# uc-vision/taichi_gaussian_rasterizer

Measured on AMD Instinct MI355X. Metric: Mpixels/s fwd+bwd @ 2048x2048, 1M Gaussians, higher is better.
Workload: dtype f32

## Files before the change

taichi_gaussian_rasterizer_amd/csrc/frame.cpp:

```cpp

#include <string.h>

#include "gs_common.h"

namespace {

int64_t a256(int64_t bytes) { return gs_align_up(bytes > 0 ? bytes : 1, 256); }

struct Dims {
  int64_t n, P, T;
  int C, F, col0, RS, tiles_x, tiles_y, local_h, D;
  bool want_vis;
};

int frame_dims(const GsFrame* f, Dims* d) {
  GS_REQUIRE(f != nullptr, GS_ERR_INVALID_ARGUMENT, "frame: descriptor is NULL");
  if (int rc = gs_check_cfg(&f->cfg)) return rc;
  GS_REQUIRE(f->n >= 0 && f->n < (int64_t(1) << 31), GS_ERR_INVALID_ARGUMENT, "frame: %lld gaussians", (long long)f->n);
  GS_REQUIRE(f->width > 0 && f->height > 0, GS_ERR_INVALID_ARGUMENT, "frame: image size %dx%d", f->width, f->height);
  GS_REQUIRE(f->sh_degree >= -1 && f->sh_degree <= 3, GS_ERR_UNSUPPORTED, "frame: SH degree %d", f->sh_degree);
  GS_REQUIRE(f->channels >= 1 && f->channels <= (f->sh_degree >= 0 ? GS_MAX_SH_CHANNELS : GS_MAX_FEATURES - 2),
             GS_ERR_UNSUPPORTED, "frame: %d feature channels", f->channels);
  const int ts = f->cfg.tile_size;
  GsShard sh;
// ... 130 lines not shown
  int32_t* tile_order = at<int32_t>(workspace, L.tile_order);
  int32_t* o2p = at<int32_t>(workspace, L.overlap_to_point);
  float* image = at<float>(workspace, L.image);
  float* alpha = at<float>(workspace, L.alpha);
  float* vis = L.visibility >= 0 ? at<float>(workspace, L.visibility) : nullptr;
  float* ndc = at<float>(scratch, L.s_ndc_depth);
  void* stage = at<char>(scratch, L.s_stage);
  const int64_t map_bytes = gs_map_scratch_bytes(d.n, d.T > 0 ? d.T : 1);
  void* proj_stage = at<char>(stage, a256(map_bytes));
  const int64_t proj_bytes = L.stage_bytes - a256(map_bytes);

  const bool lists = shard && f->exchange_world > 0 && d.T > 0;
  GS_REQUIRE(f->exchange_world <= 64 && (f->exchange_world == 0 || (f->exchange_rank >= 0 && f->exchange_rank < f->exchange_world)),
             GS_ERR_INVALID_ARGUMENT, "gs_frame_fwd: exchange rank %d of %d", f->exchange_rank, f->exchange_world);
  if (lists && f->sh_degree >= 0 &&
      hipMemsetD32Async(reinterpret_cast<hipDeviceptr_t>(feats), 0x3F000000, size_t(d.n) * d.F, s) != hipSuccess) {
    gs_set_error("gs_frame_fwd: hipMemsetD32Async failed");
    return GS_ERR_LAUNCH;
  }
  GsMapBinPlan bin;
  bin.width = f->width; bin.height = f->height; bin.cfg = cfg; bin.shard = shard; bin.scratch = stage;
  bin.scratch_bytes = map_bytes;
  tm.mark(GS_FWD_PROJECT, 0, stream);
  if (int rc = gs_project_fwd_ex(d.n, position, log_scaling, rotation, alpha_logit, T_camera_world, projection,
                                 f->width, f->height, f->near_plane, f->far_plane, cfg, points, depth, ndc, indexes,
                                 slot_of, counts, f->render_depth ? feats : nullptr, d.F, cam_pos, proj_stage,
                                 proj_bytes, L.grad_rows >= 0 ? at<float>(workspace, L.grad_rows) : nullptr, d.RS,
                                 d.T > 0 ? &bin : nullptr, stream))
    return rc;
  tm.mark(GS_FWD_PROJECT, 1, stream);
  const int32_t* v_dev = counts;
  float* colours = feats + d.col0;
  int rc;
  tm.mark(GS_FWD_COLOURS, 0, stream);
  if (f->sh_degree >= 0 && lists)
    rc = GS_OK;
  else if (f->sh_degree >= 0 && shard)
    rc = gs_sh_fwd_shard(d.n, v_dev, d.C, f->sh_degree, feature, position, indexes, cam_pos, points, f->height, cfg,
                         shard, colours, d.F, stream);
  else if (f->sh_degree >= 0)
    rc = gs_sh_fwd(d.n, v_dev, d.C, f->sh_degree, feature, position, indexes, cam_pos, colours, d.F, stream);
  else
    rc = gs_feature_gather_fwd(d.n, v_dev, d.C, feature, indexes, colours, d.F, stream);
  tm.mark(GS_FWD_COLOURS, 1, stream);
  if (rc) return rc;
  if (vis && hipMemsetAsync(vis, 0, size_t(d.n) * 4, s) != hipSuccess) {
    gs_set_error("gs_frame_fwd: hipMemsetAsync failed");
    return GS_ERR_LAUNCH;
  }
  if (d.T == 0) {
    if (hipMemsetAsync(counts + 1, 0, 28, s) != hipSuccess) { gs_set_error("gs_frame_fwd: memset failed"); return GS_ERR_LAUNCH; }
    if (L.owner_counts >= 0 && hipMemsetAsync(at<char>(workspace, L.owner_counts), 0, 64 * 8, s) != hipSuccess) {
      gs_set_error("gs_frame_fwd: memset failed");
      return GS_ERR_LAUNCH;
    }
    if (counts_host) {
      if (hipMemcpyAsync(counts_host, counts + 4, 16, hipMemcpyDeviceToHost, s) != hipSuccess ||
          hipMemcpyAsync(counts_host + 4, counts, 4, hipMemcpyDeviceToHost, s) != hipSuccess ||
          hipMemcpyAsync(counts_host + 5, counts + 5, 4, hipMemcpyDeviceToHost, s) != hipSuccess) {
        gs_set_error("gs_frame_fwd: count read-back failed");
        return GS_ERR_LAUNCH;
      }
    }
    if (counts_event && hipEventRecord(static_cast<hipEvent_t>(counts_event), s) != hipSuccess) {
      gs_set_error("gs_frame_fwd: hipEventRecord failed");
      return GS_ERR_LAUNCH;
    }
    return tm.rc;
  }
  tm.mark(GS_FWD_MAP_PREPARE, 0, stream);
  if ((rc = gs_map_prepare_ex(d.n, v_dev, points, f->width, f->height, cfg, f->k_capacity, tile_ranges, counts + 4,
                              counts_host, tile_order, shard, stage, map_bytes, 1, stream)))
    return rc;
  tm.mark(GS_FWD_MAP_PREPARE, 1, stream);
  if (counts_event && hipEventRecord(static_cast<hipEvent_t>(counts_event), s) != hipSuccess) {
    gs_set_error("gs_frame_fwd: hipEventRecord failed");
    return GS_ERR_LAUNCH;
  }
  if (lists) {
    int32_t* touched = at<int32_t>(workspace, L.touched);
    if ((rc = gs_map_touched_list(d.n, v_dev, d.T, stage, map_bytes, touched, counts + 1, indexes, d.n,
                                  f->exchange_world, at<int64_t>(workspace, L.owner_counts), f->exchange_rank,
                                  counts + 2, stream)))
      return rc;
    if (f->sh_degree >= 0) {
      tm.mark(GS_FWD_COLOURS, 0, stream);
      if ((rc = gs_sh_fwd_rows(d.n, touched, counts + 1, d.C, f->sh_degree, feature, position, indexes, cam_pos, colours,
                               d.F, stream)))
        return rc;
      tm.mark(GS_FWD_COLOURS, 1, stream);
    }
  }
  const int32_t tile_hint = f->max_tile_hint > 0 ? -f->max_tile_hint : 0;
  tm.mark(GS_FWD_MAP_FINISH, 0, stream);
  if ((rc = gs_map_finish(d.n, v_dev, f->k_capacity, tile_hint, points, ndc, f->width, f->height, cfg, f->use_depth16,
                          tile_ranges, o2p, nullptr, at<char>(scratch, L.s_pairs), shard, stage, map_bytes,
                          stream)))
    return rc;
  tm.mark(GS_FWD_MAP_FINISH, 1, stream);
  tm.mark(GS_FWD_RASTER, 0, stream);
  if ((rc = gs_raster_fwd(d.n, d.F, points, feats, tile_ranges, o2p, f->k_capacity, f->width, f->height, &rcfg,
                          tile_order, counts + 7, image, alpha, vis, shard, stream)))
    return rc;
  tm.mark(GS_FWD_RASTER, 1, stream);
  if (f->render_depth &&
// ... 101 lines not shown
```

taichi_gaussian_rasterizer_amd/csrc/gs_common.h:

```cpp
#pragma once

#include <hip/hip_runtime.h>
#include <stdint.h>
#include <stdio.h>

#include "../../include/gsplat_hip.h"

#define GS_WAVE 64

void gs_set_error(const char* fmt, ...);

#define GS_REQUIRE(cond, status, ...)  \
  do {                                 \
    if (!(cond)) {                     \
      gs_set_error(__VA_ARGS__);       \
      return (status);                 \
    }                                  \
  } while (0)

#define GS_CHECK_LAUNCH(name)                                                   \
  do {                                                                          \
    hipError_t e_ = hipGetLastError();                                          \
    if (e_ != hipSuccess) {                                                     \
      gs_set_error("%s: launch failed: %s", name, hipGetErrorString(e_));       \
// ... 73 lines not shown

int gs_raster_sub_blocks(const GsRasterConfig* cfg, int64_t num_tiles, int backward);

int gs_project_fwd_ex(int64_t n, const float* position, const float* log_scaling, const float* rotation,
                      const float* alpha_logit, const float* T_camera_world, const float* projection, int32_t width,
                      int32_t height, double near_plane, double far_plane, const GsRasterConfig* cfg, float* points,
                      float* depth, float* ndc_depth, int64_t* indexes, int32_t* slot_of, int32_t* num_visible,
                      float* depth_features, int32_t depth_features_stride, float* camera_pos, void* scratch,
                      int64_t scratch_bytes, float* zero_rows, int32_t zero_row_floats, const struct GsMapBinPlan* bin,
                      void* stream);
struct GsMapBinPlan {
  int32_t width, height;
  const GsRasterConfig* cfg;
  const GsRowShard* shard;
  void* scratch;
  int64_t scratch_bytes;
};
struct GsCompactArgs {
  int64_t n;
  const void* st_rows;
  const int* block_offsets;
  const int* block_counts;
  int num_blocks;
  float inv_far, ndc_denom;
  float* points; float* depth; float* ndc; int64_t* indexes; int* slot_of; int* num_visible;
  float* depth_feat; int depth_feat_stride;
  void* zero_rows; int zero_row_v4;
};
int gs_map_compact_bin(const GsMapBinPlan* plan, const GsCompactArgs* c, void* stream);
int gs_map_bin_counters(const GsMapBinPlan* plan, int64_t n, int32_t** words, int32_t* count);
int64_t gs_map_one_pass_scratch_bytes(int64_t n);
int gs_map_project_compact_bin(const GsMapBinPlan* plan, const void* pa, const GsCompactArgs* c, float* camera_pos,
                               void* lookback, void* stream);
int gs_map_prepare_ex(int64_t v, const int32_t* v_dev, const float* points, int32_t width, int32_t height,
                      const GsRasterConfig* cfg, int64_t k_capacity, int32_t* tile_ranges, int32_t* counts_out,
                      int32_t* counts_host, int32_t* tile_order, const GsRowShard* shard, void* scratch,
                      int64_t scratch_bytes, int binned, void* stream);
int gs_rows_add(int64_t v, int32_t row_floats, float* rows, const float* add_points, const float* add_depth,
                int32_t depth_col, void* stream);

#ifdef __HIPCC__

__device__ __forceinline__ int gs_xcd_remap(int block, int n) {
  const int chunk = (n + 7) >> 3;
  const int item = (block & 7) * chunk + (block >> 3);
  return ((block >> 3) < chunk && item < n) ? item : -1;
}

template <int CTRL, int ROW_MASK = 0xf, int BANK_MASK = 0xf>
__device__ __forceinline__ float gs_dpp_add(float x) {
  const int moved = __builtin_amdgcn_update_dpp(0, __float_as_int(x), CTRL, ROW_MASK, BANK_MASK, false);
  return x + __int_as_float(moved);
}

__device__ __forceinline__ float gs_wave_sum_to_lane63(float x) {
  x = gs_dpp_add<0x128>(x);
  x = gs_dpp_add<0x124>(x);
  x = gs_dpp_add<0x122>(x);
  x = gs_dpp_add<0x121>(x);
  x = gs_dpp_add<0x142, 0xa>(x);
  x = gs_dpp_add<0x143, 0xc>(x);
  return x;
}

template <int CTRL>
__device__ __forceinline__ float gs_dpp_add_full(float x) {
  return x + __int_as_float(__builtin_amdgcn_mov_dpp(__float_as_int(x), CTRL, 0xf, 0xf, true));
}

__device__ __forceinline__ float gs_wave_reduce16_transposed(float (&v)[16], int lane) {
// ... 176 lines not shown
```

taichi_gaussian_rasterizer_amd/csrc/mapper.hip:

```cpp

#include "gs_common.h"
#include "../../include/gs_detmath.h"
#include "project_math.h"

namespace {

struct GridQuery {
  float ib00, ib01, ib10, ib11;
  float rel_min_x, rel_min_y;
  int min_tx, min_ty, span_x, span_y;
};

__device__ __forceinline__ GridQuery grid_query(const float* g, int Wp, int Hp, int tile_size, float alpha_thr) {
  GridQuery q;
  const float mx = g[0], my = g[1], ax = g[2], ay = g[3], sgx = g[4], sgy = g[5], alpha = g[6];
  if (!(alpha > alpha_thr)) {
    q.ib00 = q.ib01 = q.ib10 = q.ib11 = q.rel_min_x = q.rel_min_y = 0.f;
    q.min_tx = q.min_ty = q.span_x = q.span_y = 0;
    return q;
  }
  const float gscale = gs_det_sqrtf(2.0f * gs_det_logf(__fdiv_rn(alpha, alpha_thr)));
  const float sx = sgx * gscale, sy = sgy * gscale;
  const float a2x = -ay, a2y = ax;
  const float v1x = ax * sx, v1y = ay * sx, v2x = a2x * sy, v2y = a2y * sy;
  const float ex = gs_det_sqrtf(v1x * v1x + v2x * v2x), ey = gs_det_sqrtf(v1y * v1y + v2y * v2y);
  const float lox = mx - ex, loy = my - ey, hix = mx + ex, hiy = my + ey;
  q.ib00 = __fdiv_rn(ax, sx); q.ib01 = __fdiv_rn(ay, sx); q.ib10 = __fdiv_rn(a2x, sy); q.ib11 = __fdiv_rn(a2y, sy);
  const float ts = float(tile_size);
  const int max_tx = (Wp - 1) / tile_size, max_ty = (Hp - 1) / tile_size;
  int min_tx = int(floorf(__fdiv_rn(lox, ts))), min_ty = int(floorf(__fdiv_rn(loy, ts)));
  min_tx = max(min_tx, 0); min_ty = max(min_ty, 0);
  int hi_tx = int(ceilf(__fdiv_rn(hix, ts))), hi_ty = int(ceilf(__fdiv_rn(hiy, ts)));
  hi_tx = min(max(hi_tx, min_tx + 1), max_tx + 1);
  hi_ty = min(max(hi_ty, min_ty + 1), max_ty + 1);
  q.min_tx = min_tx; q.min_ty = min_ty;
  q.span_x = max(hi_tx - min_tx, 0); q.span_y = max(hi_ty - min_ty, 0);
// ... 45 lines not shown
__device__ __forceinline__ int64_t live_count(const MapArgs& a) {
  if (a.v_dev == nullptr) return a.v;
  const int64_t d = *a.v_dev;
  return d < a.v ? d : a.v;
}

__device__ __forceinline__ int wave_inclusive_scan(int x) {
  x += __builtin_amdgcn_update_dpp(0, x, 0x111, 0xf, 0xf, true);
  x += __builtin_amdgcn_update_dpp(0, x, 0x112, 0xf, 0xf, true);
  x += __builtin_amdgcn_update_dpp(0, x, 0x114, 0xf, 0xf, true);
  x += __builtin_amdgcn_update_dpp(0, x, 0x118, 0xf, 0xf, true);
  x += __builtin_amdgcn_update_dpp(0, x, 0x142, 0xa, 0xf, false);
  x += __builtin_amdgcn_update_dpp(0, x, 0x143, 0xc, 0xf, false);
  return x;
}

__device__ __forceinline__ int block_exclusive_scan(int x, int* s_wave, int& sum) {
  const int lane = threadIdx.x & 63, wv = threadIdx.x >> 6;
  const int inc = wave_inclusive_scan(x);
  if (lane == 63) s_wave[wv] = inc;
  __syncthreads();
  int before = 0;
  sum = 0;
#pragma unroll
  for (int w = 0; w < 16; ++w) {
    const int tot = s_wave[w];
    sum += tot;
    before += w < wv ? tot : 0;
  }
  __syncthreads();
  return before + inc - x;
}

__global__ __launch_bounds__(1024) void map_scan_kernel(int num_tiles, const int* tile_hist, int2* tile_ranges,
                                                        int* cursors, int* counts_out, int64_t k_capacity,
                                                        int* tile_order, const int* v_dev, int* counts_host,
                                                        const int* touched_dev) {
  __shared__ int s_wave[16];
  __shared__ int s_bin[1024];
  const int t = threadIdx.x;
  if (blockIdx.x == 0) {
    constexpr int PER = 16;
    int carry = 0, mx = 0;
    for (int base0 = 0; base0 < num_tiles; base0 += 1024 * PER) {
      const int i0 = base0 + t * PER;
      int c[PER];
      const bool whole = i0 + PER <= num_tiles;
      if (whole) {
        const int4* src = reinterpret_cast<const int4*>(tile_hist + i0);
#pragma unroll
        for (int q = 0; q < PER / 4; ++q) {
          const int4 v4 = src[q];
          c[4 * q] = v4.x; c[4 * q + 1] = v4.y; c[4 * q + 2] = v4.z; c[4 * q + 3] = v4.w;
        }
      } else {
#pragma unroll
        for (int j = 0; j < PER; ++j) c[j] = i0 + j < num_tiles ? tile_hist[i0 + j] : 0;
      }
      int sum = 0;
#pragma unroll
      for (int j = 0; j < PER; ++j) { sum += c[j]; mx = max(mx, c[j]); }
      int total;
      int run = carry + block_exclusive_scan(sum, s_wave, total);
      carry += total;
      int2 rg[PER];
      int cur[PER];
#pragma unroll
      for (int j = 0; j < PER; ++j) {
        const bool fits = k_capacity <= 0 || int64_t(run) + c[j] <= k_capacity;
        rg[j] = (c[j] > 0 && fits) ? make_int2(run, run + c[j]) : make_int2(0, 0);
// ... 130 lines not shown
__device__ __forceinline__ void publish_region_hist(const int* s_hist, const RegionGrid& rg, int num_wg, int blk,
                                                    int* part, int* region_count) {
  for (int r = threadIdx.x; r < rg.num_regions; r += BIN) {
    const int h = s_hist[r];
    if (region_count == nullptr) part[int64_t(r) * num_wg + blk] = h;
    else if (h > 0) part[int64_t(r) * num_wg + blk] = atomicAdd(region_count + r, h);
  }
}
__global__ __launch_bounds__(BIN) void region_count_kernel(MapArgs a, RegionGrid rg, int num_wg, int* region_of,
                                                           int* part, int* touched_blocks, int* block_start,
                                                           int* region_count) {
  __shared__ int s_hist[MAX_REGIONS];
  for (int r = threadIdx.x; r < rg.num_regions; r += BIN) s_hist[r] = 0;
  __syncthreads();
  const int64_t i = int64_t(blockIdx.x) * BIN + threadIdx.x;
  bool mine = false;
  const int64_t live = live_count(a);
  if (threadIdx.x == 0) {
    block_start[blockIdx.x] = int(min(int64_t(blockIdx.x) * BIN, live));
    if (int(blockIdx.x) == num_wg - 1) block_start[num_wg] = int(live);
  }
  if (i < live) {
    const bool any = enters_order(a.points + 7 * i, a);
    const int r = any ? region_of_gaussian(a.points + 7 * i, a, rg) : -1;
    region_of[i] = r;
    if (r >= 0) atomicAdd(&s_hist[r], 1);
    mine = r >= 0;
  }
  const int touched = __syncthreads_count(mine);
  if (threadIdx.x == 0) touched_blocks[blockIdx.x] = touched;
  publish_region_hist(s_hist, rg, num_wg, blockIdx.x, part, region_count);
}

__global__ __launch_bounds__(1024) void region_part_scan_kernel(int num_wg, int* part, int* region_count,
                                                                int) {
  __shared__ int s_wave[16];
  int* row = part + int64_t(blockIdx.x) * num_wg;
  int carry = 0;
  for (int base = 0; base < num_wg; base += 1024) {
    const int i = base + threadIdx.x;
    const int v = i < num_wg ? row[i] : 0;
    int total;
    const int before = block_exclusive_scan(v, s_wave, total);
    if (i < num_wg) row[i] = carry + before;
    carry += total;
  }
  if (threadIdx.x == 0) region_count[blockIdx.x] = carry;
}

__global__ __launch_bounds__(1024) void region_scan_kernel(int num_regions, const int* region_count, int* region_start,
                                                           int* chunk_start) {
  __shared__ int s_wave[16];
  const int r = threadIdx.x;
  const int c = r < num_regions ? region_count[r] : 0;
  const int ch = (c + CHUNK - 1) / CHUNK;
  int total_c, total_ch;
  const int start = block_exclusive_scan(c, s_wave, total_c);
  const int chunk = block_exclusive_scan(ch, s_wave, total_ch);
  if (r < num_regions) {
    region_start[r] = start;
    chunk_start[r] = chunk;
  }
  if (r == 0) {
    region_start[num_regions] = total_c;
    chunk_start[num_regions] = total_ch;
  }
}

__global__ __launch_bounds__(BIN) void region_scatter_kernel(RegionGrid rg, int num_wg, const int* region_of,
                                                             const int* part, const int* region_count,
                                                             int* region_start, int* chunk_start,
                                                             const int* block_start, int* order, int* tile_hist,
                                                             int num_tiles, int scanned) {
  __shared__ int s_cnt[MAX_REGIONS];
  __shared__ int s_start[MAX_REGIONS];
  __shared__ int s_wave[16];
  for (int i = blockIdx.x * BIN + threadIdx.x; i < num_tiles; i += gridDim.x * BIN) tile_hist[i] = 0;
  const int t = threadIdx.x;
  s_cnt[t] = 0;
  if (scanned) {
    s_start[t] = t < rg.num_regions ? region_start[t] : 0;
  } else {
    const int c = t < rg.num_regions ? region_count[t] : 0;
    int total_c;
// ... 1075 lines not shown
  const MapScratch m = carve(plan->scratch, c->n, num_tiles);
  const unsigned vb = unsigned(gs_div_up(c->n, BIN));
  hipStream_t s = static_cast<hipStream_t>(stream);
  int* counters = bin_with_atomics(vb, rg) ? m.region_count : nullptr;
  if (counters && hipMemsetAsync(counters, 0, size_t(MAX_REGIONS + 1) * 4, s) != hipSuccess) {
    gs_set_error("gs_map_project_compact_bin: hipMemsetAsync failed");
    return GS_ERR_LAUNCH;
  }
  if (c->block_offsets == reinterpret_cast<const int*>(1)) {
    GsCompactArgs c2 = *c;
    c2.block_offsets = nullptr;
    c2.block_counts = static_cast<int*>(lookback);
    hipLaunchKernelGGL(project_count_kernel, dim3(vb), dim3(BIN), 0, s, *static_cast<const gs_proj::ProjArgs*>(pa),
                       static_cast<int*>(lookback));
    hipLaunchKernelGGL(project_compact_bin_kernel<false>, dim3(vb), dim3(BIN), 0, s,
                       *static_cast<const gs_proj::ProjArgs*>(pa), c2, a, rg, int(vb), m.region_of, m.part,
                       m.touched_blocks, m.block_start, counters, nullptr, nullptr, nullptr, camera_pos);
    GS_CHECK_LAUNCH("gs_map_project_compact_bin");
    return GS_OK;
  }
  if (hipMemsetAsync(lookback, 0, size_t(gs_map_one_pass_scratch_bytes(c->n)), s) != hipSuccess) {
    gs_set_error("gs_map_project_compact_bin: hipMemsetAsync failed");
    return GS_ERR_LAUNCH;
  }
  unsigned long long* desc = static_cast<unsigned long long*>(lookback);
  int* ticket = reinterpret_cast<int*>(desc + vb);
  hipLaunchKernelGGL(project_compact_bin_kernel<true>, dim3(vb), dim3(BIN), 0, s,
                     *static_cast<const gs_proj::ProjArgs*>(pa), *c, a, rg, int(vb), m.region_of, m.part,
                     m.touched_blocks, m.block_start, counters, desc, ticket, ticket + 1, camera_pos);
  GS_CHECK_LAUNCH("gs_map_project_compact_bin");
  return GS_OK;
}

extern "C" int gs_map_prepare(int64_t v, const int32_t* v_dev, const float* points, int32_t width, int32_t height,
                              const GsRasterConfig* cfg, int64_t k_capacity, int32_t* tile_ranges,
                              int32_t* counts_out, int32_t* counts_host, int32_t* tile_order,
                              const GsRowShard* shard, void* scratch, int64_t scratch_bytes, void* stream) {
  return gs_map_prepare_ex(v, v_dev, points, width, height, cfg, k_capacity, tile_ranges, counts_out, counts_host,
                           tile_order, shard, scratch, scratch_bytes, 0, stream);
}

int gs_map_prepare_ex(int64_t v, const int32_t* v_dev, const float* points, int32_t width, int32_t height,
                      const GsRasterConfig* cfg, int64_t k_capacity, int32_t* tile_ranges, int32_t* counts_out,
                      int32_t* counts_host, int32_t* tile_order, const GsRowShard* shard, void* scratch,
                      int64_t scratch_bytes, int binned, void* stream) {
  MapArgs a;
  if (int rc = fill_args(a, v, points, nullptr, width, height, cfg, 0, shard)) return rc;
  a.v_dev = v_dev;
  GS_REQUIRE(a.sh.local_rows > 0, GS_ERR_INVALID_ARGUMENT, "gs_map_prepare: the shard owns no tile row");
  const int num_tiles = a.tiles_wide * a.sh.local_rows;
  GS_REQUIRE(tile_ranges && counts_out && scratch, GS_ERR_INVALID_ARGUMENT, "gs_map_prepare: NULL buffer");
  GS_REQUIRE(scratch_bytes >= gs_map_scratch_bytes(v, num_tiles), GS_ERR_SCRATCH_TOO_SMALL,
             "gs_map_prepare: scratch %lld < %lld bytes", (long long)scratch_bytes,
             (long long)gs_map_scratch_bytes(v, num_tiles));
  GS_REQUIRE(num_tiles <= (1 << 20), GS_ERR_UNSUPPORTED, "gs_map_prepare: %d tiles (limit 2^20)", num_tiles);
  hipStream_t s = static_cast<hipStream_t>(stream);
  const MapScratch m = carve(scratch, v, num_tiles);
  int* hist = m.hist;
  int* cursors = m.cursors;
  const RegionGrid rg = make_grid(a);
  GS_REQUIRE(rg.num_regions <= MAX_REGIONS && rg.win * rg.win * 8 <= 65536, GS_ERR_UNSUPPORTED,
             "gs_map_prepare: tile grid %dx%d needs %d regions of edge %d", rg.tiles_x, rg.tiles_y, rg.num_regions,
             rg.rg);
  if (v == 0 && hipMemsetAsync(hist, 0, size_t(num_tiles) * 4, s) != hipSuccess) {
    gs_set_error("gs_map_prepare: hipMemsetAsync failed");
    return GS_ERR_LAUNCH;
  }
  if (v > 0) {
    GS_REQUIRE(points, GS_ERR_INVALID_ARGUMENT, "gs_map_prepare: points is NULL");
    const unsigned vb = unsigned(gs_div_up(v, BIN));
    const bool atomics = bin_with_atomics(vb, rg);
    if (!binned) {
      if (atomics && hipMemsetAsync(m.region_count, 0, size_t(MAX_REGIONS + 1) * 4, s) != hipSuccess) {
        gs_set_error("gs_map_prepare: hipMemsetAsync failed");
        return GS_ERR_LAUNCH;
      }
      hipLaunchKernelGGL(region_count_kernel, dim3(vb), dim3(BIN), 0, s, a, rg, int(vb), m.region_of, m.part,
                         m.touched_blocks, m.block_start, atomics ? m.region_count : nullptr);
    }
    if (!atomics) {
      hipLaunchKernelGGL(region_part_scan_kernel, dim3(rg.num_regions), dim3(1024), 0, s, int(vb), m.part,
                         m.region_count, 0);
      hipLaunchKernelGGL(region_scan_kernel, dim3(1), dim3(1024), 0, s, rg.num_regions, m.region_count,
                         m.region_start, m.chunk_start);
    }
    hipLaunchKernelGGL(region_scatter_kernel, dim3(vb), dim3(BIN), 0, s, rg, int(vb), m.region_of, m.part,
                       m.region_count, m.region_start, m.chunk_start, m.block_start, m.order, hist, num_tiles,
                       atomics ? 0 : 1);
    hipLaunchKernelGGL(count_binned_kernel, dim3(unsigned(gs_div_up(v, CHUNK)) + unsigned(rg.num_regions)), dim3(CHUNK),
                       size_t(rg.win) * rg.win * 4, s, a, rg, m.order,
                       m.region_start, m.chunk_start, hist, m.qcache);
    GS_CHECK_LAUNCH("gs_map_prepare/count");
  }
  hipLaunchKernelGGL(map_scan_kernel, dim3(tile_order ? 2 : 1), dim3(1024), 0, s, num_tiles, hist,
                     reinterpret_cast<int2*>(tile_ranges), cursors, counts_out, k_capacity, tile_order, v_dev,
                     counts_host, v > 0 ? m.region_start + rg.num_regions : nullptr);
  GS_CHECK_LAUNCH("gs_map_prepare/scan");
  return GS_OK;
}

extern "C" int gs_map_finish(int64_t v, const int32_t* v_dev, int64_t k, int32_t max_tile_count, const float* points,
                             const float* depth, int32_t width, int32_t height, const GsRasterConfig* cfg,
                             int32_t use_depth16, const int32_t* tile_ranges, int32_t* overlap_to_point,
                             uint64_t* sorted_keys, void* pair_scratch, const GsRowShard* shard, void* scratch,
                             int64_t scratch_bytes, void* stream) {
  MapArgs a;
  if (int rc = fill_args(a, v, points, depth, width, height, cfg, use_depth16, shard)) return rc;
  a.v_dev = v_dev;
  if (k == 0 || v == 0) return GS_OK;
  const int num_tiles = a.tiles_wide * a.sh.local_rows;
  GS_REQUIRE(points && depth && tile_ranges && overlap_to_point && pair_scratch && scratch, GS_ERR_INVALID_ARGUMENT,
             "gs_map_finish: NULL buffer");
  GS_REQUIRE(scratch_bytes >= gs_map_scratch_bytes(v, num_tiles), GS_ERR_SCRATCH_TOO_SMALL,
             "gs_map_finish: scratch too small");
  hipStream_t s = static_cast<hipStream_t>(stream);
  const MapScratch m = carve(scratch, v, num_tiles);
  int* cursors = m.cursors;
  const RegionGrid rg = make_grid(a);
  uint64_t* pairs = static_cast<uint64_t*>(pair_scratch);
  hipLaunchKernelGGL(emit_binned_kernel, dim3(unsigned(gs_div_up(v, CHUNK)) + unsigned(rg.num_regions)), dim3(CHUNK),
                     size_t(rg.win) * rg.win * 8, s,
                     a, rg, m.order, m.region_start, m.chunk_start, cursors, pairs, m.qcache);
  GS_CHECK_LAUNCH("gs_map_finish/emit");
  const int grid = 8 * int(gs_div_up(num_tiles, 8));
  const int2* r = reinterpret_cast<const int2*>(tile_ranges);
  const bool exact = max_tile_count > 0;
  const int guess = exact ? max_tile_count : (max_tile_count < 0 ? -max_tile_count : 1024);
  const bool big_pass = guess > 512;
  const int skip_full = (exact || big_pass) ? 1 : 0;
// ... 146 lines not shown
```

taichi_gaussian_rasterizer_amd/csrc/sh.hip:

```cpp

#include "gs_common.h"

namespace {

constexpr float C1 = 0.48860251190292f, C2 = 1.09254843059208f, C3 = 0.94617469575756f, C4 = 0.31539156525252f,
                C5 = 0.54627421529604f, C6 = 0.590043589926644f, C7 = 2.89061144264055f, C8 = 0.304697199642977f,
                C9 = 1.24392110863372f, C10 = 0.497568443453487f, C11 = 1.44530572132028f;

template <int DEG>
__device__ __forceinline__ void rsh(float x, float y, float z, float* Y) {
  Y[0] = 0.282094791773878f;
  if (DEG >= 1) { Y[1] = -C1 * y; Y[2] = C1 * z; Y[3] = -C1 * x; }
  if (DEG >= 2) {
    Y[4] = C2 * (x * y); Y[5] = -C2 * (y * z); Y[6] = C3 * (z * z) - C4; Y[7] = -C2 * (x * z);
    Y[8] = C5 * (x * x) - C5 * (y * y);
  }
  if (DEG >= 3) {
    const float x2 = x * x, y2 = y * y, z2 = z * z;
    Y[9] = -C6 * y * (3.0f * x2 - y2);
    Y[10] = C7 * (x * y) * z;
    Y[11] = C8 * y * (1.5f - 7.5f * z2);
    Y[12] = C9 * z * (1.5f * z2 - 0.5f) - C10 * z;
    Y[13] = C8 * x * (1.5f - 7.5f * z2);
    Y[14] = C11 * z * (x2 - y2);
    Y[15] = -C6 * x * (x2 - 3.0f * y2);
  }
}

template <int DEG>
__device__ __forceinline__ void rsh_grad(float x, float y, float z, const float* w, float* g) {
  g[0] = g[1] = g[2] = 0.0f;
  if (DEG >= 1) { g[1] += -C1 * w[1]; g[2] += C1 * w[2]; g[0] += -C1 * w[3]; }
  if (DEG >= 2) {
    g[0] += C2 * y * w[4];            g[1] += C2 * x * w[4];
    g[1] += -C2 * z * w[5];           g[2] += -C2 * y * w[5];
    g[2] += 2.0f * C3 * z * w[6];
    g[0] += -C2 * z * w[7];           g[2] += -C2 * x * w[7];
    g[0] += 2.0f * C5 * x * w[8];     g[1] += -2.0f * C5 * y * w[8];
  }
  if (DEG >= 3) {
    const float x2 = x * x, y2 = y * y, z2 = z * z;
    g[0] += -6.0f * C6 * x * y * w[9];          g[1] += -C6 * (3.0f * x2 - 3.0f * y2) * w[9];
    g[0] += C7 * y * z * w[10];                 g[1] += C7 * x * z * w[10];            g[2] += C7 * x * y * w[10];
    g[1] += C8 * (1.5f - 7.5f * z2) * w[11];    g[2] += -15.0f * C8 * y * z * w[11];
    g[2] += (C9 * (4.5f * z2 - 0.5f) - C10) * w[12];
    g[0] += C8 * (1.5f - 7.5f * z2) * w[13];    g[2] += -15.0f * C8 * x * z * w[13];
    g[0] += 2.0f * C11 * x * z * w[14];         g[1] += -2.0f * C11 * y * z * w[14];   g[2] += C11 * (x2 - y2) * w[14];
    g[0] += -C6 * (3.0f * x2 - 3.0f * y2) * w[15];  g[1] += 6.0f * C6 * x * y * w[15];
  }
}

template <int D>
__device__ __forceinline__ void load_row(const float* row, float* out) {
  if ((D & 3) == 0) {
    const float4* r4 = reinterpret_cast<const float4*>(row);
#pragma unroll
    for (int k = 0; k < D / 4; ++k) {
      const float4 t = r4[k];
      out[4 * k] = t.x; out[4 * k + 1] = t.y; out[4 * k + 2] = t.z; out[4 * k + 3] = t.w;
    }
  } else {
#pragma unroll
    for (int k = 0; k < D; ++k) out[k] = row[k];
  }
}

#ifndef GS_SH_ROW_MARGIN
#define GS_SH_ROW_MARGIN 2
#endif
struct ShTouch {
  const int* rows;
  const int* rows_count;
  const float* points2d;
  GsShard sh;
  float inv_tile, thr;
  int tile_rows;
};

__device__ __forceinline__ bool sh_touched(const ShTouch& t, int64_t i) {
  const float* g = t.points2d + i * 7;
  const float my = g[1], ax = g[2], ay = g[3], sgx = g[4], sgy = g[5], alpha = g[6];
  if (!(alpha > t.thr)) return false;
  const float gscale = sqrtf(2.0f * __logf(alpha / t.thr)) * 1.001f;
  const float v1y = ay * sgx, v2y = ax * sgy;
  const float ey = sqrtf(v1y * v1y + v2y * v2y) * gscale;
  const int lo = int(floorf((my - ey) * t.inv_tile)) - GS_SH_ROW_MARGIN, hi = int(ceilf((my + ey) * t.inv_tile)) + GS_SH_ROW_MARGIN;
  return gs_shard_any_row(t.sh, max(lo, 0), min(hi, t.tile_rows));
}

template <int DEG, int CT>
__global__ __launch_bounds__(256) void sh_fwd_kernel(int64_t v, const int* v_dev, int C, const float* params,
                                                     const float* positions, const int64_t* indexes,
                                                     const float* cam, float* out, int out_stride, const ShTouch touch) {
  constexpr int D = (DEG + 1) * (DEG + 1);
  int64_t i = int64_t(blockIdx.x) * 256 + threadIdx.x;
  if (touch.rows != nullptr) {
    if (i >= v || i >= *touch.rows_count) return;
    i = touch.rows[i];
  } else {
    if (v_dev != nullptr && i >= *v_dev) return;
    if (i >= v) return;
  }
  if (touch.points2d != nullptr && !sh_touched(touch, i)) {
    for (int c = 0; c < C; ++c) out[i * out_stride + c] = 0.5f;
    return;
  }
  const int64_t idx = indexes[i];
  if (CT > 0) {
    float rows[CT > 0 ? CT : 1][D];
#pragma unroll
    for (int c = 0; c < CT; ++c) load_row<D>(params + (idx * CT + c) * D, rows[c]);
    const float dx = positions[3 * idx] - cam[0], dy = positions[3 * idx + 1] - cam[1], dz = positions[3 * idx + 2] - cam[2];
    const float nrm = sqrtf(dx * dx + dy * dy + dz * dz);
    float Y[D];
    rsh<DEG>(dx / nrm, dy / nrm, dz / nrm, Y);
#pragma unroll
    for (int c = 0; c < CT; ++c) {
      float acc = 0.0f;
#pragma unroll
      for (int d = 0; d < D; ++d) acc += Y[d] * rows[c][d];
      out[i * out_stride + c] = fminf(fmaxf(acc + 0.5f, 0.0f), 1.0f);
    }
    return;
  }
  const float dx = positions[3 * idx] - cam[0], dy = positions[3 * idx + 1] - cam[1], dz = positions[3 * idx + 2] - cam[2];
  const float nrm = sqrtf(dx * dx + dy * dy + dz * dz);
  float Y[D];
  rsh<DEG>(dx / nrm, dy / nrm, dz / nrm, Y);
  for (int c = 0; c < C; ++c) {
    float row[D];
    load_row<D>(params + (idx * C + c) * D, row);
    float acc = 0.0f;
#pragma unroll
    for (int d = 0; d < D; ++d) acc += Y[d] * row[d];
    out[i * out_stride + c] = fminf(fmaxf(acc + 0.5f, 0.0f), 1.0f);
  }
}


template <int DEG, bool UNIQUE>
__global__ __launch_bounds__(256) void sh_bwd_kernel(int64_t v, int C, const float* params, const float* positions,
                                                     const int64_t* indexes, const float* cam, const float* gout,
                                                     float* d_params, float* d_positions, float* d_cam) {
  constexpr int D = (DEG + 1) * (DEG + 1);
  const int64_t i = int64_t(blockIdx.x) * 256 + threadIdx.x;
  float gd[3] = {0, 0, 0};
  if (i < v) {
    const int64_t idx = indexes[i];
    const float dx = positions[3 * idx] - cam[0], dy = positions[3 * idx + 1] - cam[1],
                dz = positions[3 * idx + 2] - cam[2];
    const float nrm = sqrtf(dx * dx + dy * dy + dz * dz);
    const float x = dx / nrm, y = dy / nrm, z = dz / nrm;
    float Y[D], w[D];
    rsh<DEG>(x, y, z, Y);
#pragma unroll
    for (int d = 0; d < D; ++d) w[d] = 0.0f;
    for (int c = 0; c < C; ++c) {
      float row[D];
      load_row<D>(params + (idx * C + c) * D, row);
      float acc = 0.0f;
#pragma unroll
      for (int d = 0; d < D; ++d) acc += Y[d] * row[d];
      const float pre = acc + 0.5f;
      const float g = (pre >= 0.0f && pre <= 1.0f) ? gout[i * C + c] : 0.0f;
      float* drow = d_params + (idx * C + c) * D;
#pragma unroll
      for (int d = 0; d < D; ++d) {
        if (UNIQUE) drow[d] = g * Y[d];
        else if (g != 0.0f) atomicAdd(drow + d, g * Y[d]);
// ... 148 lines not shown
  GS_REQUIRE(degree >= 0 && degree <= 3, GS_ERR_UNSUPPORTED, "%s: SH degree %d not in [0,3]", who, degree);
  GS_REQUIRE(channels >= 1 && channels <= GS_MAX_SH_CHANNELS, GS_ERR_UNSUPPORTED, "%s: %d channels", who, channels);
  if (v == 0) return GS_OK;
  GS_REQUIRE(params && positions && indexes && camera_pos && out, GS_ERR_INVALID_ARGUMENT, "%s: NULL buffer", who);
  hipStream_t s = static_cast<hipStream_t>(stream);
  if (out_stride <= 0) out_stride = channels;
  const dim3 grid(unsigned(gs_div_up(v, 256))), block(256);
#define SH_FWD_C(DEG, CT)                                                                                         \
  hipLaunchKernelGGL((sh_fwd_kernel<DEG, CT>), grid, block, 0, s, v, v_dev, channels, params, positions, indexes, \
                     camera_pos, out, out_stride, touch)
#define SH_FWD(DEG)                                                                                               \
  if (channels == 3) SH_FWD_C(DEG, 3);                                                                            \
  else SH_FWD_C(DEG, 0)
  switch (degree) {
    case 0: SH_FWD(0); break;
    case 1: SH_FWD(1); break;
    case 2: SH_FWD(2); break;
    default: SH_FWD(3); break;
  }
  GS_CHECK_LAUNCH(who);
  return GS_OK;
}
}

extern "C" int gs_sh_fwd(int64_t v, const int32_t* v_dev, int32_t channels, int32_t degree, const float* params,
                         const float* positions, const int64_t* indexes, const float* camera_pos, float* out,
                         int32_t out_stride, void* stream) {
  ShTouch touch{};
  touch.points2d = nullptr;
  return sh_fwd_launch(v, v_dev, channels, degree, params, positions, indexes, camera_pos, out, out_stride, touch,
                       stream, "gs_sh_fwd");
}

extern "C" int gs_sh_fwd_rows(int64_t v, const int32_t* rows, const int32_t* rows_count, int32_t channels,
                              int32_t degree, const float* params, const float* positions, const int64_t* indexes,
                              const float* camera_pos, float* out, int32_t out_stride, void* stream) {
  GS_REQUIRE(rows && rows_count, GS_ERR_INVALID_ARGUMENT, "gs_sh_fwd_rows: NULL row list");
  ShTouch touch{};
  touch.rows = rows;
  touch.rows_count = rows_count;
  return sh_fwd_launch(v, nullptr, channels, degree, params, positions, indexes, camera_pos, out, out_stride, touch,
                       stream, "gs_sh_fwd_rows");
}

extern "C" int gs_sh_fwd_shard(int64_t v, const int32_t* v_dev, int32_t channels, int32_t degree, const float* params,
                               const float* positions, const int64_t* indexes, const float* camera_pos,
                               const float* points2d, int32_t height, const GsRasterConfig* cfg,
                               const GsRowShard* shard, float* out, int32_t out_stride, void* stream) {
  GS_REQUIRE(cfg && cfg->tile_size >= 1 && height >= 0, GS_ERR_INVALID_ARGUMENT, "gs_sh_fwd_shard: config / height");
  GS_REQUIRE(points2d || v == 0, GS_ERR_INVALID_ARGUMENT, "gs_sh_fwd_shard: points2d is NULL");
  ShTouch touch{};
  touch.points2d = points2d;
  touch.tile_rows = int(gs_div_up(height, cfg->tile_size));
  if (int rc = gs_make_shard(shard, touch.tile_rows, &touch.sh)) return rc;
  touch.inv_tile = 1.0f / float(cfg->tile_size);
  touch.thr = cfg->alpha_threshold;
  return sh_fwd_launch(v, v_dev, channels, degree, params, positions, indexes, camera_pos, out, out_stride, touch,
                       stream, "gs_sh_fwd_shard");
}

#define SH_BWD_LAUNCH(DEG, UNIQ)                                                                                    \
  hipLaunchKernelGGL((sh_bwd_kernel<DEG, UNIQ>), grid, block, 0, s, v, channels, params, positions, indexes,        \
                     camera_pos, grad_out, d_params, d_positions, d_camera_pos)

extern "C" int gs_sh_bwd(int64_t n, int64_t v, int32_t channels, int32_t degree, const float* params,
                         const float* positions, const int64_t* indexes, int32_t indexes_unique,
// ... 63 lines not shown
```

Baseline: 3957.

## Overlap SH colour evaluation with mapper scan kernels using spare workgroups

The separate SH forward kernel is split into shares. A slice is still run as a standalone kernel, and the remaining shares are appended as extra workgroups to the single-block or few-block scan kernels in map_prepare (mostly map_scan). This is meant to fill the idle GPU while the low-parallelism scans run and to remove part of a kernel launch. In exchange, the scan kernels gain template variants and extra register and launch-bound pressure. Load imbalance is possible if the share split is poorly tuned.

```diff
diff --git a/taichi_gaussian_rasterizer_amd/csrc/frame.cpp b/taichi_gaussian_rasterizer_amd/csrc/frame.cpp
--- a/taichi_gaussian_rasterizer_amd/csrc/frame.cpp
+++ b/taichi_gaussian_rasterizer_amd/csrc/frame.cpp
@@ -186,14 +186,23 @@
   const int32_t* v_dev = counts;
   float* colours = feats + d.col0;
   int rc;
+  const bool sh_in_mapper = f->sh_degree >= 0 && !shard && d.T > 0;
+  GsShSlice sh_slice{};
+  if (sh_in_mapper) {
+    sh_slice.params = feature; sh_slice.positions = position; sh_slice.indexes = indexes; sh_slice.cam = cam_pos;
+    sh_slice.out = colours; sh_slice.v_dev = v_dev; sh_slice.v = d.n;
+    sh_slice.channels = d.C; sh_slice.degree = f->sh_degree; sh_slice.out_stride = d.F;
+    sh_slice.lo = 0;
+    sh_slice.hi = GS_SH_SHARES - gs_map_sh_shares(&bin, d.n);
+  }
   tm.mark(GS_FWD_COLOURS, 0, stream);
   if (f->sh_degree >= 0 && lists)
     rc = GS_OK;
+  else if (sh_in_mapper)
+    rc = gs_sh_fwd_slice(&sh_slice, stream);
   else if (f->sh_degree >= 0 && shard)
     rc = gs_sh_fwd_shard(d.n, v_dev, d.C, f->sh_degree, feature, position, indexes, cam_pos, points, f->height, cfg,
                          shard, colours, d.F, stream);
-  else if (f->sh_degree >= 0)
-    rc = gs_sh_fwd(d.n, v_dev, d.C, f->sh_degree, feature, position, indexes, cam_pos, colours, d.F, stream);
   else
     rc = gs_feature_gather_fwd(d.n, v_dev, d.C, feature, indexes, colours, d.F, stream);
   tm.mark(GS_FWD_COLOURS, 1, stream);
@@ -222,9 +231,13 @@
     }
     return tm.rc;
   }
+  GsShSlice map_sh = sh_slice;
+  map_sh.lo = sh_slice.hi;
+  map_sh.hi = GS_SH_SHARES;
   tm.mark(GS_FWD_MAP_PREPARE, 0, stream);
   if ((rc = gs_map_prepare_ex(d.n, v_dev, points, f->width, f->height, cfg, f->k_capacity, tile_ranges, counts + 4,
-                              counts_host, tile_order, shard, stage, map_bytes, 1, stream)))
+                              counts_host, tile_order, shard, stage, map_bytes, 1, sh_in_mapper ? &map_sh : nullptr,
+                              stream)))
     return rc;
   tm.mark(GS_FWD_MAP_PREPARE, 1, stream);
   if (counts_event && hipEventRecord(static_cast<hipEvent_t>(counts_event), s) != hipSuccess) {
diff --git a/taichi_gaussian_rasterizer_amd/csrc/gs_common.h b/taichi_gaussian_rasterizer_amd/csrc/gs_common.h
--- a/taichi_gaussian_rasterizer_amd/csrc/gs_common.h
+++ b/taichi_gaussian_rasterizer_amd/csrc/gs_common.h
@@ -129,10 +129,24 @@
 int64_t gs_map_one_pass_scratch_bytes(int64_t n);
 int gs_map_project_compact_bin(const GsMapBinPlan* plan, const void* pa, const GsCompactArgs* c, float* camera_pos,
                                void* lookback, void* stream);
+#define GS_SH_SHARES 1024
+struct GsShSlice {
+  const float* params;
+  const float* positions;
+  const int64_t* indexes;
+  const float* cam;
+  float* out;
+  const int32_t* v_dev;
+  int64_t v;
+  int32_t channels, degree, out_stride;
+  int32_t lo, hi;
+};
+int gs_sh_fwd_slice(const GsShSlice* s, void* stream);
+int gs_map_sh_shares(const GsMapBinPlan* plan, int64_t n);
 int gs_map_prepare_ex(int64_t v, const int32_t* v_dev, const float* points, int32_t width, int32_t height,
                       const GsRasterConfig* cfg, int64_t k_capacity, int32_t* tile_ranges, int32_t* counts_out,
                       int32_t* counts_host, int32_t* tile_order, const GsRowShard* shard, void* scratch,
-                      int64_t scratch_bytes, int binned, void* stream);
+                      int64_t scratch_bytes, int binned, const GsShSlice* sh, void* stream);
 int gs_rows_add(int64_t v, int32_t row_floats, float* rows, const float* add_points, const float* add_depth,
                 int32_t depth_col, void* stream);
 
diff --git a/taichi_gaussian_rasterizer_amd/csrc/mapper.hip b/taichi_gaussian_rasterizer_amd/csrc/mapper.hip
--- a/taichi_gaussian_rasterizer_amd/csrc/mapper.hip
+++ b/taichi_gaussian_rasterizer_amd/csrc/mapper.hip
@@ -2,6 +2,7 @@
 #include "gs_common.h"
 #include "../../include/gs_detmath.h"
 #include "project_math.h"
+#include "sh_math.h"
 
 namespace {
 
@@ -113,10 +114,21 @@
   return before + inc - x;
 }
 
+template <int SHV>
+__device__ __forceinline__ bool sh_spare_workgroup(const GsShSlice& sh, int grid0) {
+  if (SHV == 0 || int(blockIdx.x) < grid0) return false;
+  const int64_t i = gs_sh::slice_row(sh, int64_t(blockIdx.x) - grid0, 1024, threadIdx.x);
+  if (i >= 0) gs_sh::slice_row_fwd<SHV == 0 ? 1 : SHV>(sh, i);
+  return true;
+}
+#define GS_SH_VARIANTS(K) {&K<0>, &K<1>, &K<2>, &K<3>, &K<4>, &K<5>, &K<6>, &K<7>, &K<8>}
+
+template <int SHV>
 __global__ __launch_bounds__(1024) void map_scan_kernel(int num_tiles, const int* tile_hist, int2* tile_ranges,
                                                         int* cursors, int* counts_out, int64_t k_capacity,
                                                         int* tile_order, const int* v_dev, int* counts_host,
-                                                        const int* touched_dev) {
+                                                        const int* touched_dev, int grid0, const GsShSlice sh) {
+  if (sh_spare_workgroup<SHV>(sh, grid0)) return;
   __shared__ int s_wave[16];
   __shared__ int s_bin[1024];
   const int t = threadIdx.x;
@@ -313,8 +325,10 @@
   publish_region_hist(s_hist, rg, num_wg, blockIdx.x, part, region_count);
 }
 
+template <int SHV>
 __global__ __launch_bounds__(1024) void region_part_scan_kernel(int num_wg, int* part, int* region_count,
-                                                                int) {
+                                                                int num_regions, const GsShSlice sh) {
+  if (sh_spare_workgroup<SHV>(sh, num_regions)) return;
   __shared__ int s_wave[16];
   int* row = part + int64_t(blockIdx.x) * num_wg;
   int carry = 0;
@@ -329,8 +343,10 @@
   if (threadIdx.x == 0) region_count[blockIdx.x] = carry;
 }
 
+template <int SHV>
 __global__ __launch_bounds__(1024) void region_scan_kernel(int num_regions, const int* region_count, int* region_start,
-                                                           int* chunk_start) {
+                                                           int* chunk_start, const GsShSlice sh) {
+  if (sh_spare_workgroup<SHV>(sh, 1)) return;
   __shared__ int s_wave[16];
   const int r = threadIdx.x;
   const int c = r < num_regions ? region_count[r] : 0;
@@ -1472,18 +1488,53 @@
   return GS_OK;
 }
 
+#ifndef GS_SH_SHARE_PART_SCAN
+#define GS_SH_SHARE_PART_SCAN 0
+#endif
+#ifndef GS_SH_SHARE_REGION_SCAN
+#define GS_SH_SHARE_REGION_SCAN 0
+#endif
+#ifndef GS_SH_SHARE_MAP_SCAN
+#define GS_SH_SHARE_MAP_SCAN 192
+#endif
+namespace {
+struct ShShares {
+  int part_scan, region_scan, map_scan;
+};
+ShShares sh_shares(int64_t v, const RegionGrid& rg) {
+  if (bin_with_atomics(gs_div_up(v > 0 ? v : 1, BIN), rg)) return {0, 0, GS_SH_SHARE_MAP_SCAN};
+  return {GS_SH_SHARE_PART_SCAN, GS_SH_SHARE_REGION_SCAN, GS_SH_SHARE_MAP_SCAN};
+}
+GsShSlice take_shares(GsShSlice* sh, int shares, unsigned* blocks) {
+  GsShSlice t = *sh;
+  t.hi = sh->lo + shares < sh->hi ? sh->lo + shares : sh->hi;
+  sh->lo = t.hi;
+  *blocks = unsigned(gs_div_up(gs_div_up(t.v * (t.hi - t.lo), GS_SH_SHARES), 1024));
+  return t;
+}
+}
+
+int gs_map_sh_shares(const GsMapBinPlan* plan, int64_t n) {
+  MapArgs a;
+  if (fill_args(a, n, nullptr, nullptr, plan->width, plan->height, plan->cfg, 0, plan->shard) || a.sh.local_rows <= 0)
+    return 0;
+  const ShShares k = sh_shares(n, make_grid(a));
+  const int total = k.part_scan + k.region_scan + k.map_scan;
+  return total < GS_SH_SHARES ? total : GS_SH_SHARES;
+}
+
 extern "C" int gs_map_prepare(int64_t v, const int32_t* v_dev, const float* points, int32_t width, int32_t height,
                               const GsRasterConfig* cfg, int64_t k_capacity, int32_t* tile_ranges,
                               int32_t* counts_out, int32_t* counts_host, int32_t* tile_order,
                               const GsRowShard* shard, void* scratch, int64_t scratch_bytes, void* stream) {
   return gs_map_prepare_ex(v, v_dev, points, width, height, cfg, k_capacity, tile_ranges, counts_out, counts_host,
-                           tile_order, shard, scratch, scratch_bytes, 0, stream);
+                           tile_order, shard, scratch, scratch_bytes, 0, nullptr, stream);
 }
 
 int gs_map_prepare_ex(int64_t v, const int32_t* v_dev, const float* points, int32_t width, int32_t height,
                       const GsRasterConfig* cfg, int64_t k_capacity, int32_t* tile_ranges, int32_t* counts_out,
                       int32_t* counts_host, int32_t* tile_order, const GsRowShard* shard, void* scratch,
-                      int64_t scratch_bytes, int binned, void* stream) {
+                      int64_t scratch_bytes, int binned, const GsShSlice* sh, void* stream) {
   MapArgs a;
   if (int rc = fill_args(a, v, points, nullptr, width, height, cfg, 0, shard)) return rc;
   a.v_dev = v_dev;
@@ -1502,6 +1553,18 @@
   GS_REQUIRE(rg.num_regions <= MAX_REGIONS && rg.win * rg.win * 8 <= 65536, GS_ERR_UNSUPPORTED,
              "gs_map_prepare: tile grid %dx%d needs %d regions of edge %d", rg.tiles_x, rg.tiles_y, rg.num_regions,
              rg.rg);
+  GsShSlice rest{};
+  if (sh != nullptr) {
+    GS_REQUIRE(sh->v_dev && sh->v <= v && sh->lo >= 0 && sh->lo <= sh->hi && sh->hi <= GS_SH_SHARES,
+               GS_ERR_INVALID_ARGUMENT, "gs_map_prepare: bad SH slice");
+    rest = *sh;
+  }
+  const ShShares share = sh_shares(v, rg);
+  const int shv = sh != nullptr ? gs_sh::variant(sh->degree, sh->channels) : 0;
+  static decltype(&region_part_scan_kernel<0>) const part_scan_k[9] = GS_SH_VARIANTS(region_part_scan_kernel);
+  static decltype(&region_scan_kernel<0>) const region_scan_k[9] = GS_SH_VARIANTS(region_scan_kernel);
+  static decltype(&map_scan_kernel<0>) const map_scan_k[9] = GS_SH_VARIANTS(map_scan_kernel);
+  unsigned sh_blocks = 0;
   if (v == 0 && hipMemsetAsync(hist, 0, size_t(num_tiles) * 4, s) != hipSuccess) {
     gs_set_error("gs_map_prepare: hipMemsetAsync failed");
     return GS_ERR_LAUNCH;
@@ -1519,10 +1582,12 @@
                          m.touched_blocks, m.block_start, atomics ? m.region_count : nullptr);
     }
     if (!atomics) {
-      hipLaunchKernelGGL(region_part_scan_kernel, dim3(rg.num_regions), dim3(1024), 0, s, int(vb), m.part,
-                         m.region_count, 0);
-      hipLaunchKernelGGL(region_scan_kernel, dim3(1), dim3(1024), 0, s, rg.num_regions, m.region_count,
-                         m.region_start, m.chunk_start);
+      const GsShSlice part_sh = take_shares(&rest, share.part_scan, &sh_blocks);
+      hipLaunchKernelGGL(part_scan_k[shv], dim3(unsigned(rg.num_regions) + sh_blocks), dim3(1024), 0, s,
+                         int(vb), m.part, m.region_count, rg.num_regions, part_sh);
+      const GsShSlice region_sh = take_shares(&rest, share.region_scan, &sh_blocks);
+      hipLaunchKernelGGL(region_scan_k[shv], dim3(1 + sh_blocks), dim3(1024), 0, s, rg.num_regions, m.region_count,
+                         m.region_start, m.chunk_start, region_sh);
     }
     hipLaunchKernelGGL(region_scatter_kernel, dim3(vb), dim3(BIN), 0, s, rg, int(vb), m.region_of, m.part,
                        m.region_count, m.region_start, m.chunk_start, m.block_start, m.order, hist, num_tiles,
@@ -1532,9 +1597,11 @@
                        m.region_start, m.chunk_start, hist, m.qcache);
     GS_CHECK_LAUNCH("gs_map_prepare/count");
   }
-  hipLaunchKernelGGL(map_scan_kernel, dim3(tile_order ? 2 : 1), dim3(1024), 0, s, num_tiles, hist,
+  const GsShSlice scan_sh = take_shares(&rest, GS_SH_SHARES, &sh_blocks);
+  const int scan_grid = tile_order ? 2 : 1;
+  hipLaunchKernelGGL(map_scan_k[shv], dim3(unsigned(scan_grid) + sh_blocks), dim3(1024), 0, s, num_tiles, hist,
                      reinterpret_cast<int2*>(tile_ranges), cursors, counts_out, k_capacity, tile_order, v_dev,
-                     counts_host, v > 0 ? m.region_start + rg.num_regions : nullptr);
+                     counts_host, v > 0 ? m.region_start + rg.num_regions : nullptr, scan_grid, scan_sh);
   GS_CHECK_LAUNCH("gs_map_prepare/scan");
   return GS_OK;
 }
diff --git a/taichi_gaussian_rasterizer_amd/csrc/sh.hip b/taichi_gaussian_rasterizer_amd/csrc/sh.hip
--- a/taichi_gaussian_rasterizer_amd/csrc/sh.hip
+++ b/taichi_gaussian_rasterizer_amd/csrc/sh.hip
@@ -1,31 +1,10 @@
 
 #include "gs_common.h"
+#include "sh_math.h"
 
 namespace {
 
-constexpr float C1 = 0.48860251190292f, C2 = 1.09254843059208f, C3 = 0.94617469575756f, C4 = 0.31539156525252f,
-                C5 = 0.54627421529604f, C6 = 0.590043589926644f, C7 = 2.89061144264055f, C8 = 0.304697199642977f,
-                C9 = 1.24392110863372f, C10 = 0.497568443453487f, C11 = 1.44530572132028f;
-
-template <int DEG>
-__device__ __forceinline__ void rsh(float x, float y, float z, float* Y) {
-  Y[0] = 0.282094791773878f;
-  if (DEG >= 1) { Y[1] = -C1 * y; Y[2] = C1 * z; Y[3] = -C1 * x; }
-  if (DEG >= 2) {
-    Y[4] = C2 * (x * y); Y[5] = -C2 * (y * z); Y[6] = C3 * (z * z) - C4; Y[7] = -C2 * (x * z);
-    Y[8] = C5 * (x * x) - C5 * (y * y);
-  }
-  if (DEG >= 3) {
-    const float x2 = x * x, y2 = y * y, z2 = z * z;
-    Y[9] = -C6 * y * (3.0f * x2 - y2);
-    Y[10] = C7 * (x * y) * z;
-    Y[11] = C8 * y * (1.5f - 7.5f * z2);
-    Y[12] = C9 * z * (1.5f * z2 - 0.5f) - C10 * z;
-    Y[13] = C8 * x * (1.5f - 7.5f * z2);
-    Y[14] = C11 * z * (x2 - y2);
-    Y[15] = -C6 * x * (x2 - 3.0f * y2);
-  }
-}
+using namespace gs_sh;
 
 template <int DEG>
 __device__ __forceinline__ void rsh_grad(float x, float y, float z, const float* w, float* g) {
@@ -47,21 +26,6 @@
     g[0] += C8 * (1.5f - 7.5f * z2) * w[13];    g[2] += -15.0f * C8 * x * z * w[13];
     g[0] += 2.0f * C11 * x * z * w[14];         g[1] += -2.0f * C11 * y * z * w[14];   g[2] += C11 * (x2 - y2) * w[14];
     g[0] += -C6 * (3.0f * x2 - 3.0f * y2) * w[15];  g[1] += 6.0f * C6 * x * y * w[15];
-  }
-}
-
-template <int D>
-__device__ __forceinline__ void load_row(const float* row, float* out) {
-  if ((D & 3) == 0) {
-    const float4* r4 = reinterpret_cast<const float4*>(row);
-#pragma unroll
-    for (int k = 0; k < D / 4; ++k) {
-      const float4 t = r4[k];
-      out[4 * k] = t.x; out[4 * k + 1] = t.y; out[4 * k + 2] = t.z; out[4 * k + 3] = t.w;
-    }
-  } else {
-#pragma unroll
-    for (int k = 0; k < D; ++k) out[k] = row[k];
   }
 }
 
@@ -92,7 +56,6 @@
 __global__ __launch_bounds__(256) void sh_fwd_kernel(int64_t v, const int* v_dev, int C, const float* params,
                                                      const float* positions, const int64_t* indexes,
                                                      const float* cam, float* out, int out_stride, const ShTouch touch) {
-  constexpr int D = (DEG + 1) * (DEG + 1);
   int64_t i = int64_t(blockIdx.x) * 256 + threadIdx.x;
   if (touch.rows != nullptr) {
     if (i >= v || i >= *touch.rows_count) return;
@@ -105,36 +68,7 @@
     for (int c = 0; c < C; ++c) out[i * out_stride + c] = 0.5f;
     return;
   }
-  const int64_t idx = indexes[i];
-  if (CT > 0) {
-    float rows[CT > 0 ? CT : 1][D];
-#pragma unroll
-    for (int c = 0; c < CT; ++c) load_row<D>(params + (idx * CT + c) * D, rows[c]);
-    const float dx = positions[3 * idx] - cam[0], dy = positions[3 * idx + 1] - cam[1], dz = positions[3 * idx + 2] - cam[2];
-    const float nrm = sqrtf(dx * dx + dy * dy + dz * dz);
-    float Y[D];
-    rsh<DEG>(dx / nrm, dy / nrm, dz / nrm, Y);
-#pragma unroll
-    for (int c = 0; c < CT; ++c) {
-      float acc = 0.0f;
-#pragma unroll
-      for (int d = 0; d < D; ++d) acc += Y[d] * rows[c][d];
-      out[i * out_stride + c] = fminf(fmaxf(acc + 0.5f, 0.0f), 1.0f);
-    }
-    return;
-  }
-  const float dx = positions[3 * idx] - cam[0], dy = positions[3 * idx + 1] - cam[1], dz = positions[3 * idx + 2] - cam[2];
-  const float nrm = sqrtf(dx * dx + dy * dy + dz * dz);
-  float Y[D];
-  rsh<DEG>(dx / nrm, dy / nrm, dz / nrm, Y);
-  for (int c = 0; c < C; ++c) {
-    float row[D];
-    load_row<D>(params + (idx * C + c) * D, row);
-    float acc = 0.0f;
-#pragma unroll
-    for (int d = 0; d < D; ++d) acc += Y[d] * row[d];
-    out[i * out_stride + c] = fminf(fmaxf(acc + 0.5f, 0.0f), 1.0f);
-  }
+  fwd_row<DEG, CT>(i, C, params, positions, indexes, cam, out, out_stride);
 }
 
 
@@ -349,6 +283,29 @@
                        stream, "gs_sh_fwd");
 }
 
+namespace {
+template <int VAR>
+__global__ __launch_bounds__(256) void sh_fwd_slice_kernel(const GsShSlice s) {
+  const int64_t i = gs_sh::slice_row(s, blockIdx.x, 256, threadIdx.x);
+  if (i >= 0) gs_sh::slice_row_fwd<VAR>(s, i);
+}
+decltype(&sh_fwd_slice_kernel<1>) const sh_fwd_slice_kernels[8] = {
+    &sh_fwd_slice_kernel<1>, &sh_fwd_slice_kernel<2>, &sh_fwd_slice_kernel<3>, &sh_fwd_slice_kernel<4>,
+    &sh_fwd_slice_kernel<5>, &sh_fwd_slice_kernel<6>, &sh_fwd_slice_kernel<7>, &sh_fwd_slice_kernel<8>};
+}
+
+int gs_sh_fwd_slice(const GsShSlice* s, void* stream) {
+  GS_REQUIRE(s && s->degree >= 0 && s->degree <= 3 && s->channels >= 1 && s->channels <= GS_MAX_SH_CHANNELS &&
+                 s->lo >= 0 && s->lo <= s->hi && s->hi <= GS_SH_SHARES && s->v_dev,
+             GS_ERR_INVALID_ARGUMENT, "gs_sh_fwd_slice: bad slice");
+  const int64_t rows = gs_div_up(s->v * (s->hi - s->lo), GS_SH_SHARES);
+  if (rows == 0) return GS_OK;
+  hipLaunchKernelGGL(sh_fwd_slice_kernels[gs_sh::variant(s->degree, s->channels) - 1], dim3(unsigned(gs_div_up(rows, 256))), dim3(256), 0,
+                     static_cast<hipStream_t>(stream), *s);
+  GS_CHECK_LAUNCH("gs_sh_fwd_slice");
+  return GS_OK;
+}
+
 extern "C" int gs_sh_fwd_rows(int64_t v, const int32_t* rows, const int32_t* rows_count, int32_t channels,
                               int32_t degree, const float* params, const float* positions, const int64_t* indexes,
                               const float* camera_pos, float* out, int32_t out_stride, void* stream) {
diff --git a/taichi_gaussian_rasterizer_amd/csrc/sh_math.h b/taichi_gaussian_rasterizer_amd/csrc/sh_math.h
--- /dev/null
+++ b/taichi_gaussian_rasterizer_amd/csrc/sh_math.h
@@ -0,0 +1,101 @@
+#pragma once
+#include "gs_common.h"
+
+#ifdef __HIPCC__
+namespace gs_sh {
+
+constexpr float C1 = 0.48860251190292f, C2 = 1.09254843059208f, C3 = 0.94617469575756f, C4 = 0.31539156525252f,
+                C5 = 0.54627421529604f, C6 = 0.590043589926644f, C7 = 2.89061144264055f, C8 = 0.304697199642977f,
+                C9 = 1.24392110863372f, C10 = 0.497568443453487f, C11 = 1.44530572132028f;
+
+template <int DEG>
+__device__ __forceinline__ void rsh(float x, float y, float z, float* Y) {
+#pragma clang fp contract(fast)
+  Y[0] = 0.282094791773878f;
+  if (DEG >= 1) { Y[1] = -C1 * y; Y[2] = C1 * z; Y[3] = -C1 * x; }
+  if (DEG >= 2) {
+    Y[4] = C2 * (x * y); Y[5] = -C2 * (y * z); Y[6] = C3 * (z * z) - C4; Y[7] = -C2 * (x * z);
+    Y[8] = C5 * (x * x) - C5 * (y * y);
+  }
+  if (DEG >= 3) {
+    const float x2 = x * x, y2 = y * y, z2 = z * z;
+    Y[9] = -C6 * y * (3.0f * x2 - y2);
+    Y[10] = C7 * (x * y) * z;
+    Y[11] = C8 * y * (1.5f - 7.5f * z2);
+    Y[12] = C9 * z * (1.5f * z2 - 0.5f) - C10 * z;
+    Y[13] = C8 * x * (1.5f - 7.5f * z2);
+    Y[14] = C11 * z * (x2 - y2);
+    Y[15] = -C6 * x * (x2 - 3.0f * y2);
+  }
+}
+
+template <int D>
+__device__ __forceinline__ void load_row(const float* row, float* out) {
+  if ((D & 3) == 0) {
+    const float4* r4 = reinterpret_cast<const float4*>(row);
+#pragma unroll
+    for (int k = 0; k < D / 4; ++k) {
+      const float4 t = r4[k];
+      out[4 * k] = t.x; out[4 * k + 1] = t.y; out[4 * k + 2] = t.z; out[4 * k + 3] = t.w;
+    }
+  } else {
+#pragma unroll
+    for (int k = 0; k < D; ++k) out[k] = row[k];
+  }
+}
+
+template <int DEG, int CT>
+__device__ __forceinline__ void fwd_row(int64_t i, int C, const float* params, const float* positions,
+                                        const int64_t* indexes, const float* cam, float* out, int out_stride) {
+#pragma clang fp contract(fast)
+  constexpr int D = (DEG + 1) * (DEG + 1);
+  const int64_t idx = indexes[i];
+  if (CT > 0) {
+    float rows[CT > 0 ? CT : 1][D];
+#pragma unroll
+    for (int c = 0; c < CT; ++c) load_row<D>(params + (idx * CT + c) * D, rows[c]);
+    const float dx = positions[3 * idx] - cam[0], dy = positions[3 * idx + 1] - cam[1], dz = positions[3 * idx + 2] - cam[2];
+    const float nrm = sqrtf(dx * dx + dy * dy + dz * dz);
+    float Y[D];
+    rsh<DEG>(dx / nrm, dy / nrm, dz / nrm, Y);
+#pragma unroll
+    for (int c = 0; c < CT; ++c) {
+      float acc = 0.0f;
+#pragma unroll
+      for (int d = 0; d < D; ++d) acc += Y[d] * rows[c][d];
+      out[i * out_stride + c] = fminf(fmaxf(acc + 0.5f, 0.0f), 1.0f);
+    }
+    return;
+  }
+  const float dx = positions[3 * idx] - cam[0], dy = positions[3 * idx + 1] - cam[1], dz = positions[3 * idx + 2] - cam[2];
+  const float nrm = sqrtf(dx * dx + dy * dy + dz * dz);
+  float Y[D];
+  rsh<DEG>(dx / nrm, dy / nrm, dz / nrm, Y);
+  for (int c = 0; c < C; ++c) {
+    float row[D];
+    load_row<D>(params + (idx * C + c) * D, row);
+    float acc = 0.0f;
+#pragma unroll
+    for (int d = 0; d < D; ++d) acc += Y[d] * row[d];
+    out[i * out_stride + c] = fminf(fmaxf(acc + 0.5f, 0.0f), 1.0f);
+  }
+}
+
+__device__ __forceinline__ int64_t slice_row(const GsShSlice& s, int64_t block, int threads, int t) {
+  const int64_t d = *s.v_dev;
+  const int64_t v = d < s.v ? d : s.v;
+  const int64_t lo = v * s.lo / GS_SH_SHARES, hi = v * s.hi / GS_SH_SHARES;
+  const int64_t i = lo + block * threads + t;
+  return i < hi ? i : -1;
+}
+
+constexpr int variant(int degree, int channels) { return 1 + 2 * degree + (channels == 3 ? 1 : 0); }
+template <int VAR>
+__device__ __forceinline__ void slice_row_fwd(const GsShSlice& s, int64_t i) {
+  static_assert(VAR >= 1 && VAR <= 8, "SH variant");
+  fwd_row<(VAR - 1) / 2, (VAR - 1) % 2 ? 3 : 0>(i, s.channels, s.params, s.positions, s.indexes, s.cam, s.out,
+                                                   s.out_stride);
+}
+
+}
+#endif
```

Result: no change. 3989, median of 6 (+0.8%).
